# mlee03/FRE-NCtools

Hardware: AMD Instinct MI355X
Metric: exchange-cells/s (higher is better)
Workload: dtype f64; 1 GPU; C384 cubed sphere (6 tiles) -> 1440x720 lat-lon, conservative_order2: exchange-grid search + centroid pass + CSR build per step; nxgrid=4160000, parallelism=1 latitude band(s) of the target, one per GPU, world_size=1

## Files before the change

### fre-nctools_amd/csrc/xgrid_kernels.hip

```cpp
#include <algorithm>
#include "xgrid_device.h"
#ifndef FG_EXP
#define FG_EXP 0
#endif
static __shared__ double fgs_lds_tab[112 * 4];
#define FGS_TAB(k, j) fgs_lds_tab[(k) * 4 + (j)]
#include "geom.hip.h"
__device__ __forceinline__ void d_load_trig_table()
{
  for (int i = threadIdx.x; i < 112 * 4; i += blockDim.x) fgs_lds_tab[i] = FG_SINCOS_TAB[i >> 2][i & 3];
  __syncthreads();
}

#define SCAN_THREADS 256
#define SCAN_ITEMS   8
#define SCAN_CHUNK   (SCAN_THREADS * SCAN_ITEMS)
#define LB_AGG   (1ull << 62)
#define LB_INC   (2ull << 62)
#define LB_MASK  ((1ull << 62) - 1ull)
#define LB_SPIN_LIMIT (1u << 22)

__device__ __forceinline__ unsigned wave_incl_scan(unsigned v, int lane)
{
#pragma unroll
// ... 857 lines not shown
      if (nr > 0) {
        for (int k = 0; k < nwc; k++)
          if (d_rect_col_pass(R, d_rect_col(q, k), lon_in_min, lon_in_max, lon_in_avg)) { nc++; if (k < 64) cmask |= 1ull << k; }
      }
      cnt = (int)min((long)nr * nc, 0x3fffffffL);
    }
  }
  const unsigned incl = wave_incl_scan((unsigned)cnt, lane);
  const unsigned total = __shfl(incl, 63);
  const unsigned excl = incl - (unsigned)cnt;
  const int r = (int)((wave_no * 2654435761u >> 12) % (unsigned)ps.nreg);
  unsigned base = 0;
  if (lane == 0 && total) base = atomicAdd(&ps.fill[r * FG_FILL_STRIDE], total);
  base = __shfl(base, 0);
  int n_ok = 0;
  const unsigned first = base + excl;
  if (s < nsrc && !heavy) {
    const int loc0 = (int)min(first, (unsigned)ps.regcap);
    n_ok = min(cnt, ps.regcap - loc0);
    pair_beg[s] = r * ps.regcap + loc0;
    pair_cnt[s] = n_ok;
  }
  {
    const bool bigc = n_ok > CP_SMALL;
    const unsigned long long bm = __ballot(bigc);
    if (bm) {
      int qq = 0;
      if (lane == 0) qq = atomicAdd(big_cnt, __popcll(bm));
      qq = __shfl(qq, 0);
      if (bigc) big_list[qq + __popcll(bm & ((1ull << lane) - 1ull))] = s;
    }
  }
  const bool wide = nwc > 64;
  const int l0 = q.nw > 1 ? q.wb[0] - q.wa[0] + 1 : 64, l1 = q.nw > 2 ? q.wb[1] - q.wa[1] + 1 : 64;
  __syncthreads();
  wl[lane] = excl;
  wl[64 + lane] = wide ? 0u : (unsigned)nc;
  wl[2 * 64 + lane] = (unsigned)cmask; wl[3 * 64 + lane] = (unsigned)(cmask >> 32);
  wl[4 * 64 + lane] = (unsigned)q.j0;
  wl[5 * 64 + lane] = (unsigned)q.wa[0]; wl[6 * 64 + lane] = (unsigned)l0;
  wl[7 * 64 + lane] = (unsigned)(q.wa[1] - l0); wl[8 * 64 + lane] = (unsigned)(l0 + l1);
  wl[9 * 64 + lane] = (unsigned)(q.wa[2] - l0 - l1);
  __syncthreads();
  const unsigned lim = min(total, (unsigned)ps.regcap - min(base, (unsigned)ps.regcap));
  int *wsrc = ps.src + (size_t)r * ps.regcap + base, *wdst = ps.dst + (size_t)r * ps.regcap + base;
  const int s_first = s - lane;
  for (unsigned ob = 0; ob < lim; ob += 64) {
    const unsigned o = ob + lane;
    if (o >= lim || base + o >= (unsigned)ps.regcap) continue;
    int L = 0;
#pragma unroll
    for (int st = 32; st; st >>= 1) if (wl[L + st] <= o) L += st;
    const unsigned ncL = wl[64 + L];
    if (!ncL) continue;
    const unsigned t = o - wl[L], jr = t / ncL, kc = t - jr * ncL;
    const int k = d_kth_set_bit((unsigned long long)wl[2 * 64 + L] | ((unsigned long long)wl[3 * 64 + L] << 32), kc);
    const int i = k + (k < (int)wl[6 * 64 + L] ? (int)wl[5 * 64 + L] : k < (int)wl[8 * 64 + L] ? (int)wl[7 * 64 + L] : (int)wl[9 * 64 + L]);
    wsrc[o] = s_first + L;
    wdst[o] = ((int)wl[4 * 64 + L] + (int)jr) * R.nx + i;
  }
  if (wide && n_ok > 0) {
    int *psrc = ps.src + (size_t)r * ps.regcap + first, *pdst = ps.dst + (size_t)r * ps.regcap + first;
    int w = 0;
    for (int j = q.j0; j <= q.j1 && w < n_ok; j++)
      for (int k = 0; k < nwc && w < n_ok; k++) {
        const int i = d_rect_col(q, k);
        if (d_rect_col_pass(R, i, lon_in_min, lon_in_max, lon_in_avg)) { psrc[w] = s; pdst[w] = j * R.nx + i; w++; }
      }
  }
  return heavy;
}

__global__ __launch_bounds__(256, 4) void k_cell_struct2r(FgTileSet ts, const FgTile *tiles_in, FgTile *tiles_out, int ntiles, int nsrc, int ndst,
                                                        int nbS, FgCells S, double *area_out, FgRect R, const double *mask, int order, int *src_idx_f,
                                                        double *sums, unsigned *err, unsigned long long *band_keys, int cull,
                                                        int *heavy_list, int *heavy_cnt, FgPairSpace ps, int *pair_beg, int *pair_cnt,
                                                        int *big_list, int *big_cnt)
{
  __shared__ double vtile[256 * 17];
  __shared__ FgTile sh_tiles[FG_TILESET_MAX];
  static_assert(64 * RECT_WL_WORDS * sizeof(unsigned) <= 64 * 17 * sizeof(double), "a wave's share of vtile holds its candidate words");
  if (*R.bad) return;
  if (ts.n && (int)threadIdx.x < ts.n) sh_tiles[threadIdx.x] = ts.t[threadIdx.x];
  const bool isD = (int)blockIdx.x >= nbS;
  __shared__ unsigned long long sh_band[2];
  if (cull) {
    if (threadIdx.x == 0) { sh_band[0] = d_ord_key(R.lat_ax[R.ny]); sh_band[1] = ~d_ord_key(R.lat_ax[0]); }
    __syncthreads();
    band_keys = sh_band;
  }
  if (cull && !isD && band_keys[0]) {
    __syncthreads();
    const FgTile *tl0 = ts.n ? sh_tiles : tiles_in;
    const int s = blockIdx.x * 256 + threadIdx.x;
    bool keep = false;
    int idx_f = s;
    if (s < nsrc) {
      int t = 0;
      while (t + 1 < ntiles && s >= tl0[t + 1].cell_off) t++;
      const int loc = s - tl0[t].cell_off, i = loc % tl0[t].nx, j = loc / tl0[t].nx, nxp = tl0[t].nx + 1;
      if (order == 2) {
        int foff = 0;
        for (int m = 0; m < t; m++) foff += (tl0[m].nx + 2) * (tl0[m].ny + 2);
        idx_f = foff + (j + 1) * (tl0[t].nx + 2) + i + 1;
      }
      const int n0 = j * nxp + i;
      const double y0 = tl0[t].lat[n0], y1 = tl0[t].lat[n0 + 1], y2 = tl0[t].lat[n0 + nxp + 1], y3 = tl0[t].lat[n0 + nxp];
      const double lmin = fmin(fmin(y0, y1), fmin(y2, y3)), lmax = fmax(fmax(y0, y1), fmax(y2, y3));
      const double bmax = d_ord_val(band_keys[0]), bmin = d_ord_val(~band_keys[1]);
      keep = !((lmax <= bmin) || (lmin >= bmax)) || !(lmin == lmin);
    }
    if (!__syncthreads_or(keep)) {
      if (s < nsrc) {
        S.nv[s] = 0; S.area[s] = 0;
        pair_beg[s] = 0; pair_cnt[s] = 0;
        if (src_idx_f) src_idx_f[s] = idx_f;
        if (sums) { sums[s] = 0.0; sums[nsrc + s] = 0.0; sums[2 * (size_t)nsrc + s] = 0.0; }
      }
      if (ts.n && blockIdx.x == 0 && (int)threadIdx.x < ts.n) tiles_out[threadIdx.x] = sh_tiles[threadIdx.x];
      return;
    }
  }
  d_load_trig_table();
  const FgTile *tiles = ts.n ? sh_tiles : tiles_in;
  if (ts.n && blockIdx.x == 0 && (int)threadIdx.x < ts.n) tiles_out[threadIdx.x] = sh_tiles[threadIdx.x];
  if (!isD) {
    double box[5] = {0, 0, 0, 0, 0};
    int tl = 0;
    const int s0 = blockIdx.x * 256, s = s0 + threadIdx.x, lane = threadIdx.x & 63;
    const int nv = d_cell_record(tiles, ntiles, nsrc, S, err, s0, vtile, box, &tl, cull ? band_keys : nullptr);
    if (s < nsrc && sums) { sums[s] = 0.0; sums[nsrc + s] = 0.0; sums[2 * (size_t)nsrc + s] = 0.0; }
    if (s < nsrc && src_idx_f) {
      if (order != 2) src_idx_f[s] = s;
      else {
        int foff = 0;
        for (int t = 0; t < tl; t++) foff += (tiles[t].nx + 2) * (tiles[t].ny + 2);
        const int loc = s - tiles[tl].cell_off, i = loc % tiles[tl].nx, j = loc / tiles[tl].nx;
        src_idx_f[s] = foff + (j + 1) * (tiles[tl].nx + 2) + i + 1;
      }
    }
    const bool active = s < nsrc && nv > 0 && (!mask || mask[s] > 0.5);
    const bool heavy = d_rect_wave_candidates(R, ps, active, s, nsrc, (unsigned)(s >> 6), box[0], box[1], box[2], box[3], active ? S.lon_avg[s] : 0.0, pair_beg, pair_cnt,
                                              big_list, big_cnt, (unsigned *)(vtile + (threadIdx.x >> 6) * (64 * 17)));
    const unsigned long long m = __ballot(heavy);
    if (m) {
      int base = 0;
      if (lane == 0) base = atomicAdd(heavy_cnt, __popcll(m));
      base = __shfl(base, 0);
      if (heavy) heavy_list[base + __popcll(m & ((1ull << lane) - 1ull))] = s;
    }
  } else {
    const int d = ((int)blockIdx.x - nbS) * 256 + threadIdx.x;
    if (d < ndst) {
      const int j = d / R.nx, i = d - j * R.nx;
      area_out[d] = d_rect_area(R.col + (size_t)i * RECT_COLW, R.row + (size_t)j * 4);
    }
  }
}

__global__ __launch_bounds__(256) void k_polylist_records(FgPolyList P, FgCells S, int *src_idx_f, double *sums, FgRect R, int rect,
                                                           int *heavy_list, int *heavy_cnt, unsigned *err)
{
  if (rect && *R.bad) return;
  const int s = blockIdx.x * 256 + threadIdx.x, lane = threadIdx.x & 63;
  bool heavy = false;
  if (s < P.npoly) {
    const int n = P.n[s];
    double *v = S.verts + (size_t)s * 16;
    if (n < 3 || n > G_MAXV) {
      if (n > G_MAXV) atomicOr(err, G_ERRBIT_MAXV);
      S.nv[s] = 0; S.area[s] = 0; S.lat_min[s] = 0; S.lat_max[s] = 0; S.lon_min[s] = 0; S.lon_max[s] = 0; S.lon_avg[s] = 0;
      for (int k = 0; k < 16; k++) v[k] = 0.0;
    } else {
      double xmin = 0, xmax = 0, ymin = 0, ymax = 0;
      for (int k = 0; k < G_MAXV; k++) {
        const double x = (k < n) ? P.lon[(size_t)s * G_MAXV + k] : 0.0, y = (k < n) ? P.lat[(size_t)s * G_MAXV + k] : 0.0;
        v[k] = x; v[8 + k] = y;
        if (k == 0) { xmin = xmax = x; ymin = ymax = y; }
        else if (k < n) { xmin = fmin(xmin, x); xmax = fmax(xmax, x); ymin = fmin(ymin, y); ymax = fmax(ymax, y); }
      }
      if (!(ymin >= -G_HPI - 1.e-6) || !(ymax <= G_HPI + 1.e-6)) atomicOr(err, G_ERRBIT_BADLAT);
      S.nv[s] = n; S.area[s] = P.area[s]; S.lon_avg[s] = P.lon_avg[s];
      S.lat_min[s] = ymin; S.lat_max[s] = ymax; S.lon_min[s] = xmin; S.lon_max[s] = xmax;
      if (rect) heavy = d_rect_heavy(R, ymin, ymax, xmin, xmax);
    }
    if (src_idx_f) src_idx_f[s] = s;
    if (sums) { sums[s] = 0.0; sums[P.npoly + s] = 0.0; sums[2 * (size_t)P.npoly + s] = 0.0; }
  }
  if (rect) {
    const unsigned long long m = __ballot(heavy);
    if (m) {
      int base = 0;
      if (lane == 0) base = atomicAdd(heavy_cnt, __popcll(m));
      base = __shfl(base, 0);
      if (heavy) heavy_list[base + __popcll(m & ((1ull << lane) - 1ull))] = s;
    }
  }
}

__global__ __launch_bounds__(256) void k_rect_materialize(int ndst, FgRect R, FgCells D)
{
  const int d = blockIdx.x * 256 + threadIdx.x;
  if (d >= ndst) return;
  const int j = d / R.nx, i = d - j * R.nx;
  const double *c = R.col + (size_t)i * RECT_COLW;
  const double ya = R.lat_ax[j], yb = R.lat_ax[j + 1];
  D.lat_min[d] = ya; D.lat_max[d] = yb; D.lon_min[d] = c[4]; D.lon_max[d] = c[5]; D.lon_avg[d] = c[6]; D.nv[d] = 4;
  double *v = D.verts + (size_t)d * 16;
  for (int k = 0; k < 16; k++) v[k] = 0.0;
  v[0] = c[0]; v[1] = c[1]; v[2] = c[2]; v[3] = c[3];
  v[8] = ya; v[9] = ya; v[10] = yb; v[11] = yb;
}

__global__ __launch_bounds__(64) void k_candidates_rect(int nsrc, int H, FgCells S, const double *mask, FgRect R, FgPairSpace ps,
                                                         int *pair_beg, int *pair_cnt, const int *heavy_list, const int *heavy_cnt,
                                                         int *big_list, int *big_cnt)
{
  if (*R.bad) return;
  const int lane = threadIdx.x;
  if ((int)blockIdx.x < H) {
    const int nheavy = *heavy_cnt;
    for (int h = blockIdx.x; h < nheavy; h += H) {
      const int s = heavy_list[h];
      const double lon_in_min = S.lon_min[s], lon_in_max = S.lon_max[s], lon_in_avg = S.lon_avg[s];
      const RectQuery q = d_rect_query(R, S.lat_min[s], S.lat_max[s], lon_in_min, lon_in_max);
      const int nwc = d_rect_ncols(q), nr = q.j1 - q.j0 + 1;
      int nc = 0;
      for (int kb = 0; kb < nwc; kb += 64) {
        const int k = kb + lane;
        const bool pass = k < nwc && d_rect_col_pass(R, d_rect_col(q, k), lon_in_min, lon_in_max, lon_in_avg);
        nc += __popcll(__ballot(pass));
      }
      const long cnt_l = (long)nr * nc;
      const int cnt = (int)min(cnt_l, 0x7fffffffL);
      const int r = (int)(((unsigned)s * 2654435761u >> 12) % (unsigned)ps.nreg);
      unsigned base = 0;
      if (lane == 0 && cnt) base = atomicAdd(&ps.fill[r * FG_FILL_STRIDE], (unsigned)cnt);
      base = __shfl(base, 0);
      const int loc0 = (int)min(base, (unsigned)ps.regcap), n_ok = min(cnt, ps.regcap - loc0);
      const int wbase = r * ps.regcap + loc0;
      int cbase = 0;
      for (int kb = 0; kb < nwc && n_ok > 0; kb += 64) {
        const int k = kb + lane;
        int i = 0; bool pass = false;
        if (k < nwc) { i = d_rect_col(q, k); pass = d_rect_col_pass(R, i, lon_in_min, lon_in_max, lon_in_avg); }
        const unsigned long long m = __ballot(pass);
        const int at = cbase + __popcll(m & ((1ull << lane) - 1ull));
        if (pass)
          for (int jr = 0; jr < nr; jr++) {
            const long kk = (long)jr * nc + at;
            if (kk < n_ok) { ps.src[wbase + kk] = s; ps.dst[wbase + kk] = (q.j0 + jr) * R.nx + i; }
          }
        cbase += __popcll(m);
      }
      if (lane == 0) { pair_beg[s] = wbase; pair_cnt[s] = n_ok; if (n_ok > CP_SMALL) big_list[atomicAdd(big_cnt, 1)] = s; }
    }
    return;
  }
  __shared__ unsigned wl[64 * RECT_WL_WORDS];
  const int bR = (int)blockIdx.x - H;
  const int s = bR * 64 + lane;
  const bool active = s < nsrc && d_src_active(S, mask, s);
  double b[5] = {0, 0, 0, 0, 0};
  if (active) { b[0] = S.lat_min[s]; b[1] = S.lat_max[s]; b[2] = S.lon_min[s]; b[3] = S.lon_max[s]; b[4] = S.lon_avg[s]; }
  (void)d_rect_wave_candidates(R, ps, active, s, nsrc, (unsigned)bR, b[0], b[1], b[2], b[3], b[4], pair_beg, pair_cnt, big_list, big_cnt, wl);
}

struct ClipOut { double area, clon, clat; };

template <int ORDER, int S>
__device__ __forceinline__ void d_finish_pair(const double *px, const double *py, int n_out, double maskv,
                                              double area_in, double area_out, double lon_in_avg,
                                              ClipOut *o, unsigned long long *stats)
{
  double pa, clon = 0, clat = 0;
  if (ORDER == 2) d_poly_area_ctr<S>(px, py, n_out, lon_in_avg, &pa, &clon, &clat);
  else pa = d_poly_area<S>(px, py, n_out);
  double xarea = pa * maskv;
  double min_area = (area_in < area_out) ? area_in : area_out;
  double ratio = xarea / min_area;
  if (fabs(ratio - 1.e-6) < 1.e-15) atomicAdd(&stats[FG_STAT_BORDERLINE], 1ull);
  if (ratio > 1.e-6) { o->area = xarea; o->clon = clon; o->clat = clat; }
  else o->area = -2.0;
}

#ifndef CLIP_THREADS
#define CLIP_THREADS 256
#endif
#ifndef CLIP_SLOTS
#define CLIP_SLOTS 8
#endif
#ifndef CLIP_WAVES
#define CLIP_WAVES 4
#endif
#ifndef CLIP_PAD_LDS
#define CLIP_PAD_LDS 0
#endif

template <bool RECT, int T>
__device__ __forceinline__ int d_clip_quad_sh(double2 (*sh_poly)[T], const int tid, const int s, const int d,
                                              const FgCells &S, const FgCells &D, const FgRect &R, unsigned *err)
{
  constexpr int NV1 = RECT ? CLIP_SLOTS : 4;
  const int n1 = S.nv[s], n2 = RECT ? 4 : D.nv[d];
  if (n1 > NV1 || n2 > 4) return -1;

  const double *sv = S.verts + (size_t)s * 16;
  const double lon_in_avg = S.lon_avg[s];
  double x1[NV1], y1[NV1], x2[4], y2[4];
  double lon_out_avg;
  if (RECT) {
    const int j = d / R.nx, i = d - j * R.nx;
    const double *c = R.col + (size_t)i * RECT_COLW;
    const double ya = R.lat_ax[j], yb = R.lat_ax[j + 1];
    x2[0] = c[0]; x2[1] = c[1]; x2[2] = c[2]; x2[3] = c[3]; lon_out_avg = c[6];
    y2[0] = ya; y2[1] = ya; y2[2] = yb; y2[3] = yb;
  } else {
    const double *dv = D.verts + (size_t)d * 16;
#pragma unroll
    for (int k = 0; k < 4; k++) { x2[k] = dv[k]; y2[k] = dv[8 + k]; }
    lon_out_avg = D.lon_avg[d];
  }
  double shift = 0.0;
  {
    double dx = lon_out_avg - lon_in_avg;
    if (dx < -G_PI) shift = G_TPI; else if (dx > G_PI) shift = -G_TPI;
  }
  bool wrap = false;
#pragma unroll
  for (int k = 0; k < NV1; k++) {
    if (k < 4 || k < n1) { x1[k] = sv[k]; y1[k] = sv[8 + k]; } else { x1[k] = 0.0; y1[k] = 0.0; }
    if (k < n1 && (x1[k] > G_TPI || x1[k] < 0.0)) wrap = true;
  }
#pragma unroll
  for (int k = 0; k < 4; k++) if (shift != 0.0) x2[k] += shift;
  if (wrap) {
#pragma unroll
    for (int k = 0; k < NV1; k++) x1[k] = d_pimod1(x1[k]);
#pragma unroll
    for (int k = 0; k < 4; k++) x2[k] = d_pimod1(x2[k]);
  }
#pragma unroll
  for (int k = 0; k < NV1; k++) if (k < 4 || k < n1) sh_poly[k][tid] = make_double2(x1[k], y1[k]);
  const long long b0x = __double_as_longlong(x2[0]), b1x = __double_as_longlong(x2[1]);
  const long long b2x = __double_as_longlong(x2[2]), b3x = __double_as_longlong(x2[3]);
  const long long b0y = __double_as_longlong(y2[0]), b1y = __double_as_longlong(y2[1]);
  const long long b2y = __double_as_longlong(y2[2]), b3y = __double_as_longlong(y2[3]);
  auto cut = [=](int e) -> double2 {
    const long long m0 = -(long long)(e == 0), m1 = -(long long)(e == 1), m2 = -(long long)(e == 2), m3 = -(long long)(e == 3);
    return make_double2(__longlong_as_double((b0x & m0) | (b1x & m1) | (b2x & m2) | (b3x & m3)),
                        __longlong_as_double((b0y & m0) | (b1y & m1) | (b2y & m2) | (b3y & m3)));
  };
  int n_cur = n1;
  bool overflow = false, parallel = false;
  double2 e0 = cut(n2 - 1);
#if FG_EXP == 2
  for (int e = 0; e < 0; e++) {
#else
  for (int e = 0; e < n2 && n_cur > 0; e++) {
#endif
    double2 e1 = cut(e);
    const double x2_0 = e0.x, y2_0 = e0.y, x2_1 = e1.x, y2_1 = e1.y;
    double2 c[CLIP_SLOTS];
    unsigned inmask = 0u;
#pragma unroll
    for (int k = 0; k < CLIP_SLOTS; k++)
      if (k < n_cur) {
        c[k] = sh_poly[k][tid];
        inmask |= (unsigned)d_inside_edge(x2_0, y2_0, x2_1, y2_1, c[k].x, c[k].y) << k;
      }
    const unsigned full = (1u << n_cur) - 1u;
    const unsigned prevmask = ((inmask << 1) | (inmask >> (n_cur - 1))) & full;
    const unsigned tmask = inmask ^ prevmask;
    const int ncross = __popc(tmask);
    if (ncross > 2 || ncross + __popc(inmask) > CLIP_SLOTS) { overflow = true; break; }
    if (tmask) {
      const int ka = __ffs((int)tmask) - 1, kb = 31 - __clz((int)tmask);
      double2 I[2];
#pragma unroll
      for (int j = 0; j < 2; j++) {
        const int k = j ? kb : ka;
        const double2 p0 = sh_poly[k ? k - 1 : n_cur - 1][tid], p1 = sh_poly[k][tid];
        const double x1_0 = p0.x, y1_0 = p0.y, x1_1 = p1.x, y1_1 = p1.y;
        double dy1 = y1_1 - y1_0;
        double dy2 = y2_1 - y2_0;
        double dx1 = x1_1 - x1_0;
        double dx2 = x2_1 - x2_0;
        double ds1 = y1_0 * x1_1 - y1_1 * x1_0;
        double ds2 = y2_0 * x2_1 - y2_1 * x2_0;
        double determ = dy2 * dx1 - dy1 * dx2;
        if (fabs(determ) < 1.0e-30) parallel = true;
        I[j] = make_double2((dx2 * ds1 - dx1 * ds2) / determ, (dy2 * ds1 - dy1 * ds2) / determ);
      }
#pragma unroll
      for (int k = 0; k < CLIP_SLOTS; k++)
        if (k < n_cur && ((inmask >> k) & 1u))
          sh_poly[__popc(inmask & ((1u << k) - 1u)) + __popc(tmask & ((2u << k) - 1u))][tid] = c[k];
      sh_poly[__popc(inmask & ((1u << ka) - 1u))][tid] = I[0];
      sh_poly[__popc(inmask & ((1u << kb) - 1u)) + 1][tid] = I[1];
    }
    n_cur = ncross + __popc(inmask);
    e0 = e1;
  }
  if (overflow) return -1;
  if (parallel) atomicOr(err, G_ERRBIT_PARALLEL);
  return n_cur;
}

#ifndef CLIP_COMPACT
#define CLIP_COMPACT 0
#endif
__device__ __forceinline__ int d_row_slot(int *row_cnt, bool take, int d, int lane);
template <int ORDER, bool RECT>
__global__ __launch_bounds__(CLIP_THREADS) __attribute__((amdgpu_waves_per_eu(CLIP_WAVES, CLIP_WAVES))) void k_clip_quad(FgPairSpace ps, FgCells S, const double *mask, FgCells D, FgRect R,
                                                 double *tmp_area, double *tmp_clon, double *tmp_clat, int *nacc,
                                                 int *defer_list, int *defer_cnt,
                                                 unsigned long long *stats, unsigned *err, int *row_cnt, int *tmp_rowpos)
{
  constexpr int T = CLIP_THREADS;
  __shared__ double2 sh_poly[CLIP_SLOTS][T];
#if CLIP_PAD_LDS
  __shared__ char sh_pad[CLIP_PAD_LDS];
  if (nacc == (int *)16) sh_pad[threadIdx.x * 7 % CLIP_PAD_LDS] = 1;
#endif
#if CLIP_COMPACT
  __shared__ unsigned short sh_perm[T];
  __shared__ unsigned char sh_n[T];
  __shared__ int sh_wtot[T / 64];
#endif
  if (RECT && *R.bad) return;
  {
    const unsigned first = blockIdx.x * T, r = first / (unsigned)ps.regcap;
    if (first - r * (unsigned)ps.regcap >= ps.fill[r * FG_FILL_STRIDE]) return;
  }
  d_load_trig_table();
  const int tid = threadIdx.x, lane = tid & 63;
  const int p0 = blockIdx.x * T;
  bool defer = false;
  int n_cur = 0;
  if (d_pair_live(ps, p0 + tid)) {
    n_cur = d_clip_quad_sh<RECT, T>(sh_poly, tid, ps.src[p0 + tid], ps.dst[p0 + tid], S, D, R, err);
    if (n_cur < 0) { defer = true; n_cur = 0; }
    else if (n_cur == 0) ps.dst[p0 + tid] = -1;
  }
  int src = tid;
#if CLIP_COMPACT
  {
    const int wave = tid >> 6;
    const unsigned long long hm = __ballot(n_cur > 0);
    if (lane == 0) sh_wtot[wave] = __popcll(hm);
    sh_n[tid] = (unsigned char)n_cur;
    __syncthreads();
    int base = 0, total = 0;
#pragma unroll
    for (int w = 0; w < T / 64; w++) { const int c = sh_wtot[w]; if (w < wave) base += c; total += c; }
    if (n_cur > 0) sh_perm[base + __popcll(hm & ((1ull << lane) - 1ull))] = (unsigned short)tid;
    __syncthreads();
    if (tid < total) { src = sh_perm[tid]; n_cur = sh_n[src]; } else n_cur = 0;
  }
#endif
  bool below = false, acc = false;
  int s = -1, d_acc = -1;
  if (n_cur > 0) {
    const int p = p0 + src;
    s = ps.src[p];
    const int d = ps.dst[p];
    ClipOut o; o.area = -1.0; o.clon = 0; o.clat = 0;
    const double *px = (const double *)&sh_poly[0][src];
#if FG_EXP == 1
    o.area = n_cur + px[0] + px[1];
#else
    d_finish_pair<ORDER, 2 * T>(px, px + 1, n_cur, mask ? mask[s] : 1.0, S.area[s], D.area[d], S.lon_avg[s], &o, stats);
#endif
    if (o.area >= 0) {
      acc = true;
      tmp_area[p] = o.area;
      if (ORDER == 2) { tmp_clon[p] = o.clon; tmp_clat[p] = o.clat; }
      d_acc = d;
    } else {
      ps.dst[p] = -1;
      below = (o.area == -2.0);
    }
  }
  if (row_cnt) {
    const int slot = d_row_slot(row_cnt, acc, d_acc, lane);
    if (acc) tmp_rowpos[p0 + src] = slot;
  }
  if (__ballot(s >= 0)) {
    const int s_prev = __shfl_up(s, 1, 64);
    const bool head = (lane == 0) || (s != s_prev);
    const unsigned long long hm = __ballot(head), am = __ballot(acc);
    if (head && s >= 0) {
      const unsigned long long above = (lane == 63) ? 0ull : (hm >> (lane + 1)) << (lane + 1);
      const int end = above ? (__ffsll((long long)above) - 1) : 64;
      const unsigned long long upto = (end == 64) ? ~0ull : ((1ull << end) - 1ull);
      const int cnt = __popcll(am & upto & ~((1ull << lane) - 1ull));
      if (cnt) atomicAdd(&nacc[s], cnt);
    }
  }
  const unsigned long long dm = __ballot(defer), bm = __ballot(below);
  if (dm) {
    int q = 0;
    if (lane == 0) q = atomicAdd(defer_cnt, __popcll(dm));
    q = __shfl(q, 0);
    if (defer) defer_list[q + __popcll(dm & ((1ull << lane) - 1ull))] = p0 + tid;
  }
  if (bm && lane == 0) atomicAdd(&stats[FG_STAT_BELOW], (unsigned long long)__popcll(bm));
}

#define GEN_THREADS 64
#define GEN_CAP 16
template <int ORDER, bool RECT>
__global__ __launch_bounds__(GEN_THREADS) void k_clip_general(const int *defer_list, const int *defer_cnt,
                                                              const int *pair_src, int *pair_dst,
                                                              FgCells S, const double *mask, FgCells D, FgRect R,
                                                              double *tmp_area, double *tmp_clon, double *tmp_clat, int *nacc,
                                                              unsigned long long *stats, unsigned *err, int *row_cnt, int *tmp_rowpos)
{
  __shared__ double2 sh_a[GEN_CAP][GEN_THREADS];
  __shared__ double2 sh_b[GEN_CAP][GEN_THREADS];
  __shared__ double2 sh_cut[G_MAXV][GEN_THREADS];
  if (RECT && *R.bad) return;
  d_load_trig_table();
  const int tid = threadIdx.x;
  const int ndefer = *defer_cnt;
  for (int q = blockIdx.x * GEN_THREADS + tid; q < ndefer; q += gridDim.x * GEN_THREADS) {
    const int p = defer_list[q];
    const int s = pair_src[p], d = pair_dst[p];
    const int n1 = S.nv[s], n2 = RECT ? 4 : D.nv[d];
    const double *sv = S.verts + (size_t)s * 16;
    const double lon_in_avg = S.lon_avg[s];
    double dvx[G_MAXV], dvy[G_MAXV], lon_out_avg;
    if (RECT) {
      const int j = d / R.nx, i = d - j * R.nx;
      const double *c = R.col + (size_t)i * RECT_COLW;
      const double ya = R.lat_ax[j], yb = R.lat_ax[j + 1];
      dvx[0] = c[0]; dvx[1] = c[1]; dvx[2] = c[2]; dvx[3] = c[3]; lon_out_avg = c[6];
      dvy[0] = ya; dvy[1] = ya; dvy[2] = yb; dvy[3] = yb;
#pragma unroll
      for (int k = 4; k < G_MAXV; k++) { dvx[k] = 0.0; dvy[k] = 0.0; }
    } else {
      const double *dv = D.verts + (size_t)d * 16;
#pragma unroll
      for (int k = 0; k < G_MAXV; k++) { dvx[k] = dv[k]; dvy[k] = dv[8 + k]; }
      lon_out_avg = D.lon_avg[d];
    }
    double shift = 0.0;
    {
      double dx = lon_out_avg - lon_in_avg;
      if (dx < -G_PI) shift = G_TPI; else if (dx > G_PI) shift = -G_TPI;
    }
    bool wrap = false;
    for (int k = 0; k < n1; k++) { double xv = sv[k]; if (xv > G_TPI || xv < 0.0) wrap = true; }
    for (int k = 0; k < n1; k++) {
      double xv = sv[k]; if (wrap) xv = d_pimod1(xv);
      sh_a[k][tid] = make_double2(xv, sv[8 + k]);
    }
#pragma unroll
    for (int k = 0; k < G_MAXV; k++)
      if (k < n2) {
        double xv = dvx[k]; if (shift != 0.0) xv += shift; if (wrap) xv = d_pimod1(xv);
        sh_cut[k][tid] = make_double2(xv, dvy[k]);
      }
    double2 (*cur)[GEN_THREADS] = sh_a;
    double2 (*nxt)[GEN_THREADS] = sh_b;
    int n_cur = n1;
    bool overflow = false, parallel = false;
    double2 e0 = sh_cut[n2 - 1][tid];
    for (int e = 0; e < n2 && n_cur > 0 && !overflow; e++) {
      double2 e1 = sh_cut[e][tid];
      const double x2_0 = e0.x, y2_0 = e0.y, x2_1 = e1.x, y2_1 = e1.y;
      double2 lastv = cur[n_cur - 1][tid];
      double x1_0 = lastv.x, y1_0 = lastv.y;
      int inside_last = d_inside_edge(x2_0, y2_0, x2_1, y2_1, x1_0, y1_0);
      int n_new = 0;
      for (int k = 0; k < n_cur; k++) {
        double2 cv = cur[k][tid];
        double x1_1 = cv.x, y1_1 = cv.y;
        int inside = d_inside_edge(x2_0, y2_0, x2_1, y2_1, x1_1, y1_1);
        if (inside != inside_last) {
          double dy1 = y1_1 - y1_0;
          double dy2 = y2_1 - y2_0;
          double dx1 = x1_1 - x1_0;
          double dx2 = x2_1 - x2_0;
          double ds1 = y1_0 * x1_1 - y1_1 * x1_0;
          double ds2 = y2_0 * x2_1 - y2_1 * x2_0;
          double determ = dy2 * dx1 - dy1 * dx2;
          if (fabs(determ) < 1.0e-30) parallel = true;
          if (n_new < GEN_CAP) nxt[n_new][tid] = make_double2((dx2 * ds1 - dx1 * ds2) / determ,
                                                              (dy2 * ds1 - dy1 * ds2) / determ);
          else overflow = true;
          n_new++;
        }
        if (inside) {
          if (n_new < GEN_CAP) nxt[n_new][tid] = make_double2(x1_1, y1_1);
          else overflow = true;
          n_new++;
        }
        x1_0 = x1_1; y1_0 = y1_1; inside_last = inside;
      }
      n_cur = n_new;
      double2 (*t)[GEN_THREADS] = cur; cur = nxt; nxt = t;
      e0 = e1;
    }
    if (overflow) { atomicOr(err, G_ERRBIT_OVERFLOW); pair_dst[p] = -1; continue; }
    if (parallel) atomicOr(err, G_ERRBIT_PARALLEL);
    ClipOut o; o.area = -1.0; o.clon = 0; o.clat = 0;
    if (n_cur > 0) {
      const double *px = (const double *)&cur[0][tid];
      d_finish_pair<ORDER, 2 * GEN_THREADS>(px, px + 1, n_cur, mask ? mask[s] : 1.0, S.area[s], D.area[d],
                                            lon_in_avg, &o, stats);
    }
    if (o.area >= 0) {
      tmp_area[p] = o.area;
      if (ORDER == 2) { tmp_clon[p] = o.clon; tmp_clat[p] = o.clat; }
      atomicAdd(&nacc[s], 1);
      if (row_cnt) tmp_rowpos[p] = atomicAdd(&row_cnt[d], 1);
    } else {
      pair_dst[p] = -1;
      if (o.area == -2.0) atomicAdd(&stats[FG_STAT_BELOW], 1ull);
    }
  }
}

#define CP_SPAN (256 + CP_SMALL)
static_assert(CP_SMALL % 64 == 0 && CP_SMALL <= 256, "the halo lanes of k_compact are whole waves of its 256-lane block");

struct CpPair { int s, d, beg, cnt, row; long x0; int na; double a, l, t; bool mine; };

__device__ __forceinline__ int d_row_slot(int *row_cnt, bool take, int d, int lane)
{
  const int key = take ? d : -1 - lane;
  const int prev = __shfl_up(key, 1, 64);
  const bool head = (lane == 0) || (key != prev);
  const unsigned long long hm = __ballot(head), am = __ballot(take);
  int slot = 0;
  if (!am) return 0;
  if (4 * __popcll(hm & am) > 3 * __popcll(am)) {
    if (take) slot = atomicAdd(&row_cnt[d], 1);
    return slot;
  }
  unsigned long long rem = am;
  for (int it = 0; rem && it < 8; it++) {
    const int lead = __ffsll((long long)rem) - 1;
    const int d0 = __shfl(d, lead);
    const unsigned long long grp = __ballot(take && d == d0) & rem;
    int base = 0;
    if (lane == lead) base = atomicAdd(&row_cnt[d0], __popcll(grp));
    base = __shfl(base, lead);
    if ((grp >> lane) & 1ull) slot = base + __popcll(grp & ((1ull << lane) - 1ull));
    rem &= ~grp;
  }
  if ((rem >> lane) & 1ull) slot = atomicAdd(&row_cnt[d], 1);
  return slot;
}

template <int ORDER, bool HALO>
__device__ __forceinline__ void d_cp_load(const FgPairSpace &ps, const FgCompactIo &io, int p0, int tid, unsigned live_end, CpPair &c, CpPair &h)
{
  constexpr int N = HALO ? 2 : 1;
  const int *const rowpos = io.tmp_rowpos ? io.tmp_rowpos : ps.dst;
  int p[N], pc[N], s[N], d[N], rp[N], beg[N], cnt[N], rb[N], x0[N], x1[N];
  bool ok[N];
  double a[N], l[N], t[N];
#pragma unroll
  for (int k = 0; k < N; k++) { p[k] = p0 + 256 * k + tid; ok[k] = (unsigned)p[k] < live_end; pc[k] = ok[k] ? p[k] : p0; }
#pragma unroll
  for (int k = 0; k < N; k++) {
    s[k] = ps.src[pc[k]]; d[k] = ps.dst[pc[k]]; rp[k] = rowpos[pc[k]];
    if (k == 0) { a[k] = io.tmp_area[pc[k]]; if (ORDER == 2) { l[k] = io.tmp_clon[pc[k]]; t[k] = io.tmp_clat[pc[k]]; } }
  }
#pragma unroll
  for (int k = 0; k < N; k++) {
    beg[k] = io.pair_beg[s[k]]; cnt[k] = io.pair_cnt[s[k]]; rb[k] = io.row_ptr[max(d[k], 0)];
    x0[k] = io.xoff[s[k]]; x1[k] = io.xoff[s[k] + 1];
  }
#pragma unroll
  for (int k = 0; k < N; k++) {
    const bool mine = ok[k] && cnt[k] <= CP_SMALL && beg[k] >= p0 && beg[k] < p0 + 256;
    if (k == 1) {
      a[k] = 0; l[k] = 0; t[k] = 0;
      if (mine && d[k] >= 0) { a[k] = io.tmp_area[p[k]]; if (ORDER == 2) { l[k] = io.tmp_clon[p[k]]; t[k] = io.tmp_clat[p[k]]; } }
    }
    CpPair &o = k ? h : c;
    o.s = ok[k] ? s[k] : 0; o.d = ok[k] ? d[k] : -1; o.beg = ok[k] ? beg[k] : 0; o.cnt = ok[k] ? cnt[k] : 0;
    o.mine = mine; o.x0 = mine ? x0[k] : 0; o.na = mine ? x1[k] - x0[k] : 0; o.row = (int)((unsigned)rb[k] + (unsigned)rp[k]);
    o.a = a[k]; o.l = (ORDER == 2) ? l[k] : 0.0; o.t = (ORDER == 2) ? t[k] : 0.0;
  }
}

template <int ORDER>
__device__ __forceinline__ long d_cp_place(const FgCompactIo &io, const CpPair &c, int p0, const int *sh_d, double (*sh_v)[CP_SPAN])
{
  if (!c.mine || c.d < 0 || c.x0 + c.na > io.xcap) return -1;
  int rank = 0;
  const int lb = c.beg - p0;
  for (int j = 0; j < c.cnt; j++) rank += ((unsigned)sh_d[lb + j] < (unsigned)c.d) ? 1 : 0;
  const long pos = c.x0 + rank;
  io.x_src[pos] = c.s; io.x_dst[pos] = c.d; io.x_area[pos] = c.a;
  if (ORDER == 2) { io.x_c1[pos] = c.l; io.x_c2[pos] = c.t; sh_v[0][lb + rank] = c.a; sh_v[1][lb + rank] = c.l; sh_v[2][lb + rank] = c.t; }
  if (io.tmp_rowpos) io.perm[c.row] = FgRowEnt{(int)pos, c.s};
  else return pos;
  return -1;
}

#define RANK_WORDS 1024
#define BIG_STAGE 512
#define BIG_BLOCKS 512
#define CP_LDS_DOUBLES (RANK_WORDS + RANK_WORDS / 2 + 3 * BIG_STAGE)

template <int ORDER>
__device__ __forceinline__ void d_compact_big(int nsrc, const FgPairSpace &ps, const FgCompactIo &io, double *lds)
{
  unsigned long long *bits = (unsigned long long *)lds;
  int *pref = (int *)(lds + RANK_WORDS);
  double (*sval)[BIG_STAGE] = (double (*)[BIG_STAGE])(lds + RANK_WORDS + RANK_WORDS / 2);
  __shared__ int smin, smax;
  if (blockIdx.x == 0 && threadIdx.x < 64) {
    unsigned long long f = 0; unsigned mx = 0;
    for (int r = threadIdx.x; r < ps.nreg; r += 64) { const unsigned v = ps.fill[r * FG_FILL_STRIDE]; f += v; mx = max(mx, v); }
#pragma unroll
    for (int o = 32; o; o >>= 1) { f += __shfl_xor(f, o); mx = max(mx, (unsigned)__shfl_xor((int)mx, o)); }
    if (threadIdx.x == 0) { io.dc->total[1] = f; io.dc->total[3] = mx; }
  }
  const int nb = *io.big_cnt;
  for (int h = blockIdx.x; h < nb; h += BIG_BLOCKS) {
    const int s = io.big_list[h];
    const int o = io.pair_beg[s], c = io.pair_cnt[s];
    const long x0 = io.xoff[s];
    const int na = io.xoff[s + 1] - (int)x0;
    if (threadIdx.x == 0) { smin = 0x7fffffff; smax = -1; }
    __syncthreads();
    int lmin = 0x7fffffff, lmax = -1;
    for (int k = threadIdx.x; k < c; k += 256) { const int d = ps.dst[o + k]; if (d >= 0) { lmin = min(lmin, d); lmax = max(lmax, d); } }
    if (lmax >= 0) { atomicMin(&smin, lmin); atomicMax(&smax, lmax); }
    __syncthreads();
    const int dmin = smin, dmax = smax;
    const long span = (long)dmax - dmin + 1;
    const bool bitmap = dmax >= 0 && span <= (long)RANK_WORDS * 64;
    if (bitmap) {
      const int nw = (int)((span + 63) >> 6);
      for (int w = threadIdx.x; w < nw; w += 256) bits[w] = 0ull;
      __syncthreads();
      for (int k = threadIdx.x; k < c; k += 256) {
        const int d = ps.dst[o + k];
        if (d >= 0) atomicOr(&bits[(d - dmin) >> 6], 1ull << ((d - dmin) & 63));
      }
      __syncthreads();
      const int per = (nw + 255) / 256, w0 = threadIdx.x * per, w1 = min(nw, w0 + per);
      int mine = 0;
      for (int w = w0; w < w1; w++) mine += __popcll(bits[w]);
      unsigned tot;
      const int before = (int)block_incl_scan((unsigned)mine, &tot) - mine;
      int run = before;
      for (int w = w0; w < w1; w++) { pref[w] = run; run += __popcll(bits[w]); }
      __syncthreads();
    }
    const bool ahead = na <= BIG_STAGE;
    const int *const rowpos = io.tmp_rowpos ? io.tmp_rowpos : ps.dst;
    double acc = 0;
    for (int c0 = 0; c0 < max(na, 1); c0 += BIG_STAGE) {
      for (int k = threadIdx.x; k < c; k += 256) {
        const int p = o + k;
        const int d = ps.dst[p];
        double a = 0, l = 0, t = 0;
        int row = 0;
        if (ahead) {
          a = io.tmp_area[p]; if (ORDER == 2) { l = io.tmp_clon[p]; t = io.tmp_clat[p]; }
          row = (int)((unsigned)rowpos[p] + (unsigned)io.row_ptr[max(d, 0)]);
// ... 260 lines not shown
```

Measured before the change: 5.326 billion exchange-cells/s.

## Batch clip-kernel global loads up front and unroll the edge loop

Issues all source/destination vertex loads, pair indices and trig-table values early, using empty asm barriers to force them to be materialised together so memory latency overlaps instead of being serialised behind branches. Inlines the pair-liveness check and table fill, reuses loaded src/dst indices instead of rereading them, and fully unrolls the 4-edge clip loop with unconditional LDS reads of polygon slots. The risk is higher register pressure, which could cut occupancy, and extra loads for invalid or out-of-range slots.

```diff
diff --git a/fre-nctools_amd/csrc/xgrid_kernels.hip b/fre-nctools_amd/csrc/xgrid_kernels.hip
--- a/fre-nctools_amd/csrc/xgrid_kernels.hip
+++ b/fre-nctools_amd/csrc/xgrid_kernels.hip
@@ -1183,25 +1183,35 @@
                                               const FgCells &S, const FgCells &D, const FgRect &R, unsigned *err)
 {
   constexpr int NV1 = RECT ? CLIP_SLOTS : 4;
-  const int n1 = S.nv[s], n2 = RECT ? 4 : D.nv[d];
-  if (n1 > NV1 || n2 > 4) return -1;
-
   const double *sv = S.verts + (size_t)s * 16;
-  const double lon_in_avg = S.lon_avg[s];
   double x1[NV1], y1[NV1], x2[4], y2[4];
   double lon_out_avg;
+  int n1 = S.nv[s], n2 = RECT ? 4 : D.nv[d];
+  double lon_in_avg = S.lon_avg[s];
+#pragma unroll
+  for (int k = 0; k < NV1; k++) { x1[k] = sv[k]; y1[k] = sv[8 + k]; }
   if (RECT) {
     const int j = d / R.nx, i = d - j * R.nx;
     const double *c = R.col + (size_t)i * RECT_COLW;
-    const double ya = R.lat_ax[j], yb = R.lat_ax[j + 1];
+    double ya = R.lat_ax[j], yb = R.lat_ax[j + 1];
     x2[0] = c[0]; x2[1] = c[1]; x2[2] = c[2]; x2[3] = c[3]; lon_out_avg = c[6];
+    asm volatile("" : "+v"(ya), "+v"(yb));
     y2[0] = ya; y2[1] = ya; y2[2] = yb; y2[3] = yb;
   } else {
     const double *dv = D.verts + (size_t)d * 16;
 #pragma unroll
     for (int k = 0; k < 4; k++) { x2[k] = dv[k]; y2[k] = dv[8 + k]; }
     lon_out_avg = D.lon_avg[d];
-  }
+#pragma unroll
+    for (int k = 0; k < 4; k++) asm volatile("" : "+v"(y2[k]));
+    asm volatile("" : "+v"(n2));
+  }
+#pragma unroll
+  for (int k = 0; k < NV1; k++) asm volatile("" : "+v"(x1[k]), "+v"(y1[k]));
+#pragma unroll
+  for (int k = 0; k < 4; k++) asm volatile("" : "+v"(x2[k]));
+  asm volatile("" : "+v"(n1), "+v"(lon_in_avg), "+v"(lon_out_avg));
+  if (n1 > NV1 || n2 > 4) return -1;
   double shift = 0.0;
   {
     double dx = lon_out_avg - lon_in_avg;
@@ -1210,7 +1220,7 @@
   bool wrap = false;
 #pragma unroll
   for (int k = 0; k < NV1; k++) {
-    if (k < 4 || k < n1) { x1[k] = sv[k]; y1[k] = sv[8 + k]; } else { x1[k] = 0.0; y1[k] = 0.0; }
+    if (!(k < 4 || k < n1)) { x1[k] = 0.0; y1[k] = 0.0; }
     if (k < n1 && (x1[k] > G_TPI || x1[k] < 0.0)) wrap = true;
   }
 #pragma unroll
@@ -1238,18 +1248,19 @@
 #if FG_EXP == 2
   for (int e = 0; e < 0; e++) {
 #else
-  for (int e = 0; e < n2 && n_cur > 0; e++) {
+#pragma unroll
+  for (int e = 0; e < 4; e++) {
+    if ((!RECT && e >= n2) || n_cur <= 0) break;
 #endif
     double2 e1 = cut(e);
     const double x2_0 = e0.x, y2_0 = e0.y, x2_1 = e1.x, y2_1 = e1.y;
     double2 c[CLIP_SLOTS];
     unsigned inmask = 0u;
 #pragma unroll
+    for (int k = 0; k < CLIP_SLOTS; k++) c[k] = sh_poly[k][tid];
+#pragma unroll
     for (int k = 0; k < CLIP_SLOTS; k++)
-      if (k < n_cur) {
-        c[k] = sh_poly[k][tid];
-        inmask |= (unsigned)d_inside_edge(x2_0, y2_0, x2_1, y2_1, c[k].x, c[k].y) << k;
-      }
+      if (k < n_cur) inmask |= (unsigned)d_inside_edge(x2_0, y2_0, x2_1, y2_1, c[k].x, c[k].y) << k;
     const unsigned full = (1u << n_cur) - 1u;
     const unsigned prevmask = ((inmask << 1) | (inmask >> (n_cur - 1))) & full;
     const unsigned tmask = inmask ^ prevmask;
@@ -1309,18 +1320,23 @@
   __shared__ unsigned char sh_n[T];
   __shared__ int sh_wtot[T / 64];
 #endif
-  if (RECT && *R.bad) return;
-  {
-    const unsigned first = blockIdx.x * T, r = first / (unsigned)ps.regcap;
-    if (first - r * (unsigned)ps.regcap >= ps.fill[r * FG_FILL_STRIDE]) return;
-  }
-  d_load_trig_table();
   const int tid = threadIdx.x, lane = tid & 63;
   const int p0 = blockIdx.x * T;
+  const unsigned first = blockIdx.x * T, reg = first / (unsigned)ps.regcap;
+  const unsigned fill = ps.fill[reg * FG_FILL_STRIDE];
+  const unsigned bad = RECT ? *R.bad : 0u;
+  if ((RECT && bad != 0u) | (first - reg * (unsigned)ps.regcap >= fill)) return;
+  static_assert(2 * T >= 112 * 4, "at most two table values per lane");
+  const int t0 = min(tid, 112 * 4 - 1), t1 = min(tid + T, 112 * 4 - 1);
+  int s_in = ps.src[p0 + tid], d_in = ps.dst[p0 + tid];
+  double tab0 = FG_SINCOS_TAB[t0 >> 2][t0 & 3], tab1 = FG_SINCOS_TAB[t1 >> 2][t1 & 3];
+  asm volatile("" : "+v"(s_in), "+v"(d_in), "+v"(tab0), "+v"(tab1));
+  fgs_lds_tab[t0] = tab0; fgs_lds_tab[t1] = tab1;
+  __syncthreads();
   bool defer = false;
   int n_cur = 0;
-  if (d_pair_live(ps, p0 + tid)) {
-    n_cur = d_clip_quad_sh<RECT, T>(sh_poly, tid, ps.src[p0 + tid], ps.dst[p0 + tid], S, D, R, err);
+  if ((unsigned)(p0 + tid) - reg * (unsigned)ps.regcap < min(fill, (unsigned)ps.regcap)) {
+    n_cur = d_clip_quad_sh<RECT, T>(sh_poly, tid, s_in, d_in, S, D, R, err);
     if (n_cur < 0) { defer = true; n_cur = 0; }
     else if (n_cur == 0) ps.dst[p0 + tid] = -1;
   }
@@ -1344,8 +1360,8 @@
   int s = -1, d_acc = -1;
   if (n_cur > 0) {
     const int p = p0 + src;
-    s = ps.src[p];
-    const int d = ps.dst[p];
+    s = CLIP_COMPACT ? ps.src[p] : s_in;
+    const int d = CLIP_COMPACT ? ps.dst[p] : d_in;
     ClipOut o; o.area = -1.0; o.clon = 0; o.clat = 0;
     const double *px = (const double *)&sh_poly[0][src];
 #if FG_EXP == 1
```

New measurement: 5.492 billion exchange-cells/s (median of 6 runs). 3.1% higher.
